# andimarafioti/qwen3-tts-cuda-graphs

Hardware: NVIDIA B200
Metric: audio_seconds_per_second (higher is better)
Workload: dtype bf16

## Files before the change

### include/fq3.h

```cpp
#ifndef FQ3_H_
#define FQ3_H_

#include <stdint.h>

#ifdef __cplusplus
extern "C" {
#endif

#define FQ3_ABI_VERSION 2
#define FQ3_MAX_CODE_GROUPS 32

typedef struct fq3_engine fq3_engine;

typedef struct fq3_stack_desc {
  int32_t hidden, inter, n_layers, n_q_heads, n_kv_heads, head_dim, vocab;
  float rms_eps;
  const uint64_t* layer_offs;
  uint64_t final_norm_off;
  uint64_t rope_cos_off, rope_sin_off;
  int32_t rope_len;
  int32_t max_pos;
} fq3_stack_desc;

typedef struct fq3_model_desc {
// ... 66 lines not shown
int fq3_prefill_head(fq3_engine* e, int stream_idx, const void* last_hidden, int T, const fq3_policy* policy, void* out_logits,
                     void* stream);
void* fq3_kv_cache_ptr(fq3_engine* e, int stream_idx, int layer, int which);
int fq3_talker_step(fq3_engine* e, int stream_idx, const void* embeds, int position, void* out_hidden,
                    void* out_logits, void* stream);
int fq3_predictor_run(fq3_engine* e, int stream_idx, const void* pred_input, const fq3_subpolicy* sub,
                      uint64_t seed, void* out_codes_i64, void* out_logits, void* stream);
int fq3_sample(fq3_engine* e, const void* logits_f32, int V, const void* history_i64, int n_history,
               const fq3_policy* policy, int eos_id, int suppress_eos, int flags, uint64_t draw_index,
               void* out_token_i64, void* stream);
int fq3_apply_repetition_penalty(fq3_engine* e, void* logits_f32, int V, const void* history_i64, int n_history,
                                 float penalty, int flags, void* stream);
int fq3_decode_frames(fq3_engine* e, int n_streams, int n_frames, const fq3_policy* policy,
                      const fq3_subpolicy* sub, void* stream);
int fq3_assemble_prompt(fq3_engine* e, const void* tp_rows, const void* desc_i32x4, int n_rows, const void* spk_rows,
                        const void* ref_codes_i32, void* out_bf16, void* stream);
int fq3_lockstep_group(const fq3_engine* e);

int fq3_reduced_grid(const fq3_engine* e);
int fq3_set_decode_grid(fq3_engine* e, int n_ctas);
int fq3_clear_fault(fq3_engine* e, void* stream);
int fq3_debug_set_epoch(fq3_engine* e, uint32_t epoch);
int fq3_debug_read_talker_logits(fq3_engine* e, int stream_idx, void* out_f32, void* stream);
int fq3_get_status(fq3_engine* e, int stream_idx, fq3_status* out, void* stream);
int fq3_read_codes(fq3_engine* e, int stream_idx, int first_frame, int n, int32_t* codes_out, void* stream);
int fq3_last_hidden(fq3_engine* e, int row, void* out_bf16, void* stream);
void* fq3_codes_device_ptr(fq3_engine* e, int stream_idx);

int fq3_debug_read_prof(fq3_engine* e, long long* out, int n_words);

int fq3_linear(fq3_engine* e, const void* W, const void* x, void* y, int M, int N, int K, int flags,
               const void* gamma, float eps, const void* bias, const void* residual, void* stream);

enum {
  FQ3_OK = 0,
  FQ3_E_INVALID = 1,
  FQ3_E_CUDA = 2,
  FQ3_E_TOO_LONG = 3,
  FQ3_E_DEVICE_FAULT = 4,
  FQ3_E_UNSUPPORTED = 5
};

#ifdef __cplusplus
}
#endif
#endif
// ... 1 lines not shown
```

### qwen3_tts_cuda_graphs_b200/_lib.py

```python
from __future__ import annotations

import ctypes as C
import os
import shutil

from . import build as _build


class StackDesc(C.Structure):
    _fields_ = [
        ("hidden", C.c_int32), ("inter", C.c_int32), ("n_layers", C.c_int32), ("n_q_heads", C.c_int32),
        ("n_kv_heads", C.c_int32), ("head_dim", C.c_int32), ("vocab", C.c_int32), ("rms_eps", C.c_float),
        ("layer_offs", C.POINTER(C.c_uint64)), ("final_norm_off", C.c_uint64),
        ("rope_cos_off", C.c_uint64), ("rope_sin_off", C.c_uint64), ("rope_len", C.c_int32), ("max_pos", C.c_int32),
    ]


class ModelDesc(C.Structure):
    _fields_ = [
        ("abi_version", C.c_int32), ("arena", C.c_void_p), ("arena_bytes", C.c_uint64),
        ("talker", StackDesc), ("predictor", StackDesc),
        ("codec_head_off", C.c_uint64), ("codec_embed_off", C.c_uint64), ("n_code_groups", C.c_int32),
        ("lm_head_offs", C.POINTER(C.c_uint64)), ("pred_embed_offs", C.POINTER(C.c_uint64)),
        ("has_s2m", C.c_int32), ("s2m_w_off", C.c_uint64), ("s2m_b_off", C.c_uint64),
# ... 35 lines not shown
    "fq3_set_stream_policy": (C.c_int, [_P, C.c_int, C.POINTER(Policy), _P]),
    "fq3_set_generation_state": (C.c_int, [_P, C.c_int, C.c_int, C.c_int, _P]),
    "fq3_set_text_conditioning": (C.c_int, [_P, C.c_int, _P, C.c_int, _P, _P]),
    "fq3_open_text": (C.c_int, [_P, C.c_int, _P, _P]),
    "fq3_append_text": (C.c_int, [_P, C.c_int, _P, C.c_int, C.c_int, _P]),
    "fq3_import_kv": (C.c_int, [_P, C.c_int, C.c_int, _P, _P, C.c_int, _P]),
    "fq3_set_loop_state": (C.c_int, [_P, C.c_int, C.c_int, _P, C.c_int, C.c_int, _P]),
    "fq3_prefill": (C.c_int, [_P, C.c_int, _P, C.c_int, C.c_int, C.POINTER(Policy), _P, _P]),
    "fq3_prefill_tail": (C.c_int, [_P, C.c_int, _P, C.c_int, C.c_int, C.POINTER(Policy), _P, _P]),
    "fq3_prefill_head": (C.c_int, [_P, C.c_int, _P, C.c_int, C.POINTER(Policy), _P, _P]),
    "fq3_kv_cache_ptr": (_P, [_P, C.c_int, C.c_int, C.c_int]),
    "fq3_talker_step": (C.c_int, [_P, C.c_int, _P, C.c_int, _P, _P, _P]),
    "fq3_predictor_run": (C.c_int, [_P, C.c_int, _P, C.POINTER(SubPolicy), C.c_uint64, _P, _P, _P]),
    "fq3_sample": (C.c_int, [_P, _P, C.c_int, _P, C.c_int, C.POINTER(Policy), C.c_int, C.c_int, C.c_int, C.c_uint64, _P, _P]),
    "fq3_apply_repetition_penalty": (C.c_int, [_P, _P, C.c_int, _P, C.c_int, C.c_float, C.c_int, _P]),
    "fq3_decode_frames": (C.c_int, [_P, C.c_int, C.c_int, C.POINTER(Policy), C.POINTER(SubPolicy), _P]),
    "fq3_reduced_grid": (C.c_int, [_P]),
    "fq3_lockstep_group": (C.c_int, [_P]),
    "fq3_assemble_prompt": (C.c_int, [_P, _P, _P, C.c_int, _P, _P, _P, _P]),
    "fq3_set_decode_grid": (C.c_int, [_P, C.c_int]),
    "fq3_clear_fault": (C.c_int, [_P, _P]),
    "fq3_debug_set_epoch": (C.c_int, [_P, C.c_uint32]),
    "fq3_debug_read_talker_logits": (C.c_int, [_P, C.c_int, _P, _P]),
    "fq3_get_status": (C.c_int, [_P, C.c_int, C.POINTER(Status), _P]),
    "fq3_read_codes": (C.c_int, [_P, C.c_int, C.c_int, C.c_int, C.POINTER(C.c_int32), _P]),
    "fq3_last_hidden": (C.c_int, [_P, C.c_int, _P, _P]),
    "fq3_codes_device_ptr": (_P, [_P, C.c_int]),
    "fq3_debug_read_prof": (C.c_int, [_P, C.POINTER(C.c_longlong), C.c_int]),
    "fq3_linear": (C.c_int, [_P, _P, _P, _P, C.c_int, C.c_int, C.c_int, C.c_int, _P, C.c_float, _P, _P, _P]),
}

_lib = None


class Fq3Error(RuntimeError):
    pass


def load():
    global _lib
    if _lib is not None:
        return _lib
    path = _build.lib_path("libfq3.so")
    if (not os.path.exists(path) or _build.is_stale("libfq3.so")) and (shutil.which("nvcc") or os.path.exists("/usr/local/cuda/bin/nvcc")):
        _build.build_lib("libfq3.so")
    if not os.path.exists(path):
# ... 24 lines not shown
```

### qwen3_tts_cuda_graphs_b200/csrc/fq3_api.cu

```cuda
#include <cstdio>
#include <cstdlib>
#include <cstring>
#include <string>
#include <array>
#include <vector>

#include "../../include/fq3.h"
#include "fq3_kernel.cuh"

using namespace fq3;

namespace {

thread_local std::string g_err;
int fail(int code, const std::string& msg) {
  g_err = msg;
  return -code;
}
#define CK(call)                                                                                     \
  do {                                                                                               \
    cudaError_t _e = (call);                                                                         \
    if (_e != cudaSuccess)                                                                           \
      return fail(FQ3_E_CUDA, std::string(#call) + ": " + cudaGetErrorString(_e) + " @" + __FILE__ + ":" + \
                                  std::to_string(__LINE__));                                         \
// ... 39 lines not shown
  uint8_t* seen_scratch = nullptr;
  Phase *d_frames = nullptr, *d_pred = nullptr, *d_talker = nullptr, *d_prefill = nullptr, *d_linear = nullptr, *d_wide = nullptr;
  std::vector<Phase> h_frames, h_pred, h_talker, h_prefill, h_wide;
  int n_frames_ph = 0, n_pred_ph = 0, n_talker_ph = 0, n_prefill_ph = 0, n_wide_ph = 0;
  int ref_stages = 0;
  int wide_rows = 0;
  std::vector<uint8_t> in_wpin;
  uint8_t* tiled = nullptr;
  size_t tiled_bytes = 0;
  std::vector<std::pair<uint64_t, uint64_t>> tiled_map;
  uint8_t* lin_img = nullptr;
  size_t lin_img_bytes = 0;
  size_t tiled_used = 0;
  int64_t launches = 0;
  long long* prof = nullptr;
  std::vector<Plan> plans;
  int n_sms = 0;
  std::vector<std::array<int, 3>> plan_keys;
  long ring_cap = 0;
  int prof_cta = -1;
  uint32_t epoch = 1;
  int lin_words = 0;
  unsigned long long watchdog_ns = 4000000000ull;
  std::vector<void*> owned;
};

namespace {

template <class T>
int dalloc(fq3_engine* e, T** p, size_t n, bool zero = true) {
  void* q = nullptr;
  CK(cudaMalloc(&q, std::max<size_t>(n * sizeof(T), 16)));
  if (zero) CK(cudaMemset(q, 0, std::max<size_t>(n * sizeof(T), 16)));
  e->owned.push_back(q);
  *p = reinterpret_cast<T*>(q);
  return 0;
}

uint32_t off16(uint64_t byte_off) { return (uint32_t)(byte_off >> 4); }

bool make_plan(int G, int N, int K, bool swiglu, Plan* out) {
  if (N < 2 || (N & 1) || K < 64 || (K % 64)) return false;
  if (swiglu && (N & 3)) return false;
  Plan pl{};
  pl.ro_shift = swiglu ? 2 : 1;
  const int n_groups = (N + kGroupRows - 1) / kGroupRows;
// ... 37 lines not shown
  p.w_off = off16(o[1]); p.g_off = off16(o[0]); p.b_off = 0; p.N = s.qkvdim(); p.K = s.d.hidden;
  p.plan = plan_id(e, p.N, p.K, false);
  v.push_back(p);
  p.type = PH_ATTN; p.flags = r2; p.in_buf = Q; p.out_buf = A; p.w_off = 0; p.g_off = off16(o[2]); p.b_off = off16(o[3]);
  p.N = 0; p.K = 0; p.plan = 0;
  v.push_back(p);
  p.type = PH_GEMV; p.flags = F_RESID | r2 | kp; p.in_buf = A; p.out_buf = X; p.res_buf = X;
  p.w_off = off16(o[4]); p.g_off = 0; p.b_off = 0; p.N = s.d.hidden; p.K = s.qdim();
  p.plan = plan_id(e, p.N, p.K, false);
  v.push_back(p);
  p.flags = F_PRENORM | F_SWIGLU | r2 | kp; p.in_buf = X; p.out_buf = C; p.res_buf = 0;
  p.w_off = off16(o[6]); p.g_off = off16(o[5]); p.N = 2 * s.d.inter; p.K = s.d.hidden;
  p.plan = plan_id(e, p.N, p.K, true);
  v.push_back(p);
  p.flags = F_RESID | r2 | kp; p.in_buf = C; p.out_buf = X; p.res_buf = X;
  p.w_off = off16(o[7]); p.g_off = 0; p.N = s.d.hidden; p.K = s.d.inter;
  p.plan = plan_id(e, p.N, p.K, false);
  v.push_back(p);
}

void push_predictor(std::vector<Phase>& v, fq3_engine* e, bool only) {
  for (int i = 0; i < e->ncb; ++i) {
    const bool r2 = (i == 0);
    if (e->desc.has_s2m) {
      Phase p{};
      p.type = PH_GEMV; p.stack = ST_PRED; p.aux = (uint8_t)i; p.flags = F_BIAS | F_L2_KEEP | (r2 ? F_ROWS2 : 0);
      p.in_buf = BUF_PIN; p.out_buf = BUF_PX; p.w_off = off16(e->desc.s2m_w_off); p.b_off = off16(e->desc.s2m_b_off);
      p.N = e->pr.d.hidden; p.K = e->tk.d.hidden;
      p.plan = plan_id(e, p.N, p.K, false);
      v.push_back(p);
    }
    for (int l = 0; l < e->pr.d.n_layers; ++l) push_layer(e, v, e->pr, ST_PRED, l, r2, (uint8_t)i, true);
    Phase h{};
    h.type = PH_GEMV; h.stack = ST_PRED; h.aux = (uint8_t)i;
    h.flags = F_PRENORM | F_OUT_F32 | F_L2_KEEP | (r2 ? F_ROWS2 : 0);
    h.in_buf = BUF_PX; h.out_buf = BUF_LOGITS; h.w_off = off16(e->lm_head_offs[i]);
    h.g_off = off16(e->pr.d.final_norm_off); h.N = e->pr.d.vocab; h.K = e->pr.d.hidden;
    h.plan = plan_id(e, h.N, h.K, false);
    v.push_back(h);
    Phase s{};
    s.type = PH_SAMPLE; s.stack = ST_PRED; s.aux = (uint8_t)i; s.skind = only ? SMP_PRED_ONLY : SMP_PRED;
    s.flags = r2 ? F_ROWS2 : 0;
    v.push_back(s);
  }
}

void push_predictor_wide(std::vector<Phase>& v, fq3_engine* e) {
  const int L = e->pr.d.n_layers;
  for (int half = 0; half < 2; ++half) {
    const uint16_t fb = half ? F_WPIN_B : 0;
    const size_t first = v.size();
    if (e->desc.has_s2m) {
      Phase p{};
      p.type = PH_GEMV; p.stack = ST_PRED; p.aux = 0; p.flags = F_BIAS | F_L2_KEEP | F_IN_PREV | fb;
      p.in_buf = BUF_WPIN; p.out_buf = BUF_PX; p.w_off = off16(e->desc.s2m_w_off); p.b_off = off16(e->desc.s2m_b_off);
// ... 84 lines not shown
  }
  if (dalloc(e, d, v.size(), false)) return -1;
  if (cudaMemcpy(*d, v.data(), v.size() * sizeof(Phase), cudaMemcpyHostToDevice) != cudaSuccess) return -1;
  return 0;
}

void fill_common(fq3_engine* e, LaunchParams& p) {
  p.arena = reinterpret_cast<const uint8_t*>(e->desc.arena);
  p.tiled = e->tiled;
  for (int i = 0; i < kNumBufs; ++i) { p.bufs[i] = e->bufs[i]; p.ld[i] = e->ld[i]; }
  p.stacks[0] = e->rt[0];
  p.stacks[1] = e->rt[1];
  p.st = e->d_st;
  p.attn_part = e->attn_part;
  for (size_t i = 0; i < e->plans.size(); ++i) p.plans[i] = e->plans[i];
  p.err = e->err_dev;
  p.n_code_groups = e->desc.n_code_groups;
  p.eos_id = e->desc.eos_id;
  p.has_s2m = e->desc.has_s2m;
  p.max_frames = e->desc.max_frames;
  p.codec_embed = reinterpret_cast<const bf16*>(p.arena + e->desc.codec_embed_off);
  for (int i = 0; i < e->ncb; ++i) p.pred_embeds[i] = reinterpret_cast<const bf16*>(p.arena + e->pred_embed_offs[i]);
  p.pred_logits_all = nullptr;
  p.pos_override = -1;
  p.watchdog_ns = e->watchdog_ns;
  p.debug = (16 << 16) | 32;
  p.prof = e->prof;
  p.prof_cta = e->prof_cta;
  if (const char* d = getenv("FQ3_DEBUG")) p.debug = atoi(d);
  p.n_iters = 1;
  p.stream0 = 0;
  p.wide = 0;
  p.max_streams = e->desc.max_streams;
}

int check_device_fault(fq3_engine* e) {
  if (e->err_host && e->err_host[0] != 0) {
    char b[256];
    snprintf(b, sizeof b, "device watchdog fault: code=%d cta=%d phase=%d detail=%d (1=grid barrier 2=ring full-wait "
                          "3=ring empty-wait 4=frame handshake 5=bad phase)",
             e->err_host[0], e->err_host[1], e->err_host[2], e->err_host[3]);
    return fail(FQ3_E_DEVICE_FAULT, b);
  }
  return 0;
}

// ... 115 lines not shown
  Policy p{};
  p.do_sample = q->do_sample; p.top_k = q->top_k; p.top_p = q->top_p; p.temperature = q->temperature;
  p.rep_pen = q->repetition_penalty; p.min_new_tokens = q->min_new_tokens; p.suppress_tail = q->suppress_tail;
  p.seed = q->seed;
  return p;
}
SubPolicy to_sub(const fq3_subpolicy* q) {
  SubPolicy p{};
  p.do_sample = q->do_sample; p.top_k = q->top_k; p.top_p = q->top_p; p.temperature = q->temperature;
  return p;
}

int sync_pin_layout(fq3_engine* e, int s0, int n, bool to_wpin, cudaStream_t s) {
  const int pb = e->desc.has_s2m ? BUF_PIN : BUF_PX;
  for (int i = s0; i < s0 + n; ++i) {
    if ((e->in_wpin[i] != 0) == to_wpin) continue;
    fq3_wpin_from_pairs_kernel<<<1, 256, 0, s>>>(reinterpret_cast<LLWord*>(e->bufs[BUF_WPIN]), e->ld[BUF_WPIN], reinterpret_cast<LLWord*>(e->bufs[pb]),
                                                 e->ld[pb], i, e->desc.max_streams, to_wpin ? 0 : 1);
    e->launches += 1;
    CK(cudaGetLastError());
    e->in_wpin[i] = to_wpin ? 1 : 0;
  }
  return 0;
}

int check_stack(const fq3_stack_desc& d, const char* name) {
  if (d.head_dim != kHeadDim) return fail(FQ3_E_UNSUPPORTED, std::string(name) + ": head_dim must be 128");
  if (d.hidden % 64 || d.inter % 64) return fail(FQ3_E_UNSUPPORTED, std::string(name) + ": dims must be multiples of 64");
  if (d.n_q_heads % d.n_kv_heads) return fail(FQ3_E_UNSUPPORTED, std::string(name) + ": nq % nkv != 0");
  if (d.n_q_heads / d.n_kv_heads > kGq) return fail(FQ3_E_UNSUPPORTED, std::string(name) + ": more than 2 q heads per kv head");
  if (d.vocab > kMaxVocab) return fail(FQ3_E_UNSUPPORTED, std::string(name) + ": vocab exceeds sampling scratch");
  if (d.vocab % 4) return fail(FQ3_E_UNSUPPORTED, std::string(name) + ": vocab must be a multiple of 4");
  return 0;
}

}

extern "C" {

int fq3_abi_version(void) { return FQ3_ABI_VERSION; }
const char* fq3_last_error(void) { return g_err.c_str(); }

static int create_impl(const fq3_model_desc* desc, fq3_engine* e);

int fq3_create(const fq3_model_desc* desc, fq3_engine** out) {
  if (!desc || !out) return fail(FQ3_E_INVALID, "null argument");
// ... 110 lines not shown
  e->text_open.assign(B, 0);
  if (dalloc(e, &e->d_st, B)) return -FQ3_E_CUDA;
  if (dalloc(e, &e->d_spol, B)) return -FQ3_E_CUDA;
  for (int b = 0; b < B; ++b) {
    StreamState& s = e->h_st[b];
    memset(&s, 0, sizeof s);
    bf16 *tr = nullptr, *pe = nullptr;
    if (dalloc(e, &tr, (size_t)e->tk.d.max_pos * Ht)) return -FQ3_E_CUDA;
    if (dalloc(e, &pe, (size_t)Ht)) return -FQ3_E_CUDA;
    if (dalloc(e, &s.held, (size_t)Ht)) return -FQ3_E_CUDA;
    if (dalloc(e, &s.codes, (size_t)desc->max_frames * desc->n_code_groups)) return -FQ3_E_CUDA;
    if (dalloc(e, &s.seen, (size_t)round_up(e->tk.d.vocab, 16))) return -FQ3_E_CUDA;
    s.trailing = tr;
    s.pad_embed = pe;
  }
  CK(cudaMemcpy(e->d_st, e->h_st.data(), sizeof(StreamState) * B, cudaMemcpyHostToDevice));
  auto gemv_bytes = [&](const StackHost& sh) {
    return (size_t)sh.d.n_layers * ((size_t)sh.qkvdim() * sh.d.hidden + (size_t)sh.d.hidden * sh.qdim() + 3ull * sh.d.hidden * sh.d.inter) * 2;
  };
  e->tiled_bytes = gemv_bytes(e->tk) + gemv_bytes(e->pr) + (size_t)e->tk.d.vocab * e->tk.d.hidden * 2 +
                   (size_t)e->ncb * e->pr.d.vocab * e->pr.d.hidden * 2 + (desc->has_s2m ? (size_t)e->pr.d.hidden * e->tk.d.hidden * 2 : 0) +
                   1024 * (size_t)(8 * (e->tk.d.n_layers + e->pr.d.n_layers) + e->ncb + 8);
  if (dalloc(e, &e->tiled, e->tiled_bytes, false)) return -FQ3_E_CUDA;
  std::vector<Phase>& v = e->h_frames;
  push_predictor(v, e, false);
  push_talker(v, e, false);
  {
    Phase s{};
    s.type = PH_SAMPLE; s.stack = ST_TALKER; s.skind = SMP_TALKER;
    v.push_back(s);
  }
  push_predictor(e->h_pred, e, true);
  push_talker(e->h_talker, e, false);
  push_talker(e->h_prefill, e, true);
  {
    Phase s{};
    s.type = PH_SAMPLE; s.stack = ST_TALKER; s.skind = SMP_PREFILL;
    e->h_prefill.push_back(s);
  }
  push_predictor_wide(e->h_wide, e);
  push_talker(e->h_wide, e, false);
  {
    Phase s{};
    s.type = PH_SAMPLE; s.stack = ST_TALKER; s.skind = SMP_TALKER;
    e->h_wide.push_back(s);
  }
// ... 1 lines not shown
  e->n_frames_ph = (int)e->h_frames.size();
  e->n_pred_ph = (int)e->h_pred.size();
  e->n_talker_ph = (int)e->h_talker.size();
  e->n_prefill_ph = (int)e->h_prefill.size();
  e->n_wide_ph = (int)e->h_wide.size();
  if (upload(e, e->h_wide, &e->d_wide)) return fail(FQ3_E_CUDA, "wide program upload");
  {
    const int kmax = std::max(e->tk.kmax(), e->pr.kmax());
    const long fixed = kHeaderBytes + kScratchBytes + (long)round_up((size_t)kKindBytes + kUnitBytes + (size_t)e->n_wide_ph * sizeof(Phase), 1024) +
                       (long)kGammaSlots * (long)round_up((size_t)std::max(e->tk.d.hidden, e->pr.d.hidden) * 2, 1024);
    const long spg_max = ((long)kmax * 16 + kStageBytes - 1) / kStageBytes;
    const long avail = (long)e->smem_max - fixed - std::max(4L, spg_max + 1) * kStageBytes - 2048;
    e->wide_rows = (int)std::max<long>(0, std::min<long>(avail / ((long)kmax * 2 + 64), kMaxWide));
  }
  {
    LaunchParams q{};
    q.n_phases = e->n_frames_ph; q.n_rows = 1;
    if (carve(e, q, e->h_frames.data()) < 0) return -FQ3_E_INVALID;
    e->ref_stages = q.n_stages;
  }
  if (upload(e, e->h_frames, &e->d_frames) || upload(e, e->h_pred, &e->d_pred) || upload(e, e->h_talker, &e->d_talker) ||
      upload(e, e->h_prefill, &e->d_prefill))
    return fail(FQ3_E_CUDA, "program upload / weight tiling (matrix rows must be a multiple of 8)");
  if (dalloc(e, &e->d_linear, 1)) return -FQ3_E_CUDA;
  CK(cudaDeviceSynchronize());
  return 0;
}

int fq3_destroy(fq3_engine* e) {
  if (!e) return 0;
  cudaDeviceSynchronize();
  for (void* p : e->owned) if (p) cudaFree(p);
  if (e->err_host) cudaFreeHost(e->err_host);
  delete e;
  return 0;
}

int fq3_num_sms(const fq3_engine* e) { return e ? e->G : 0; }
int64_t fq3_launch_count(const fq3_engine* e) { return e ? e->launches : 0; }

static int check_stream(fq3_engine* e, int idx) {
  if (!e) return fail(FQ3_E_INVALID, "null engine");
  if (idx < 0 || idx >= e->desc.max_streams) return fail(FQ3_E_INVALID, "stream index out of range");
  return 0;
}

// ... 325 lines not shown

int fq3_decode_frames(fq3_engine* e, int n_streams, int n_frames, const fq3_policy* policy, const fq3_subpolicy* sub,
                      void* stream) {
  if (!e || !policy || !sub) return fail(FQ3_E_INVALID, "bad decode arguments");
  if (n_streams < 1 || n_streams > e->desc.max_streams) return fail(FQ3_E_INVALID, "n_streams out of range");
  if (n_frames <= 0) return 0;
  int wide_from = 3;
  if (const char* wf = getenv("FQ3_WIDE_FROM")) wide_from = std::max(1, atoi(wf));
  if ((n_streams >= wide_from && e->wide_rows > kMaxRows / 2) || 2 * n_streams > kMaxRows) {
    if (e->wide_rows <= kMaxRows / 2)
      return fail(FQ3_E_UNSUPPORTED, "more than four lock-step streams do not fit this model's staging buffer: decode in groups of fq3_lockstep_group()");
    const int n_groups = (n_streams + e->wide_rows - 1) / e->wide_rows;
    const int per = (n_streams + n_groups - 1) / n_groups;
    if (int r = sync_pin_layout(e, 0, n_streams, true, (cudaStream_t)stream)) return r;
    for (int s0 = 0; s0 < n_streams; s0 += per) {
      const int n = std::min(per, n_streams - s0);
      if (int r = reserve_epochs(e, (uint64_t)n_frames * (uint64_t)e->n_wide_ph + 2, (cudaStream_t)stream)) return r;
      LaunchParams p{};
      fill_common(e, p);
      p.prog = e->d_wide;
      p.n_phases = e->n_wide_ph;
      p.mode = MODE_FRAMES;
      p.wide = 1;
      p.n_rows = n;
      p.stream0 = s0;
      p.n_iters = n_frames;
      p.pol = to_policy(policy);
      p.spol = spol_for(e, s0, n);
      p.sub = to_sub(sub);
      if (int r = launch(e, p, e->h_wide.data(), (cudaStream_t)stream)) return r;
    }
    return 0;
  }
  if (int r = reserve_epochs(e, (uint64_t)n_frames * (uint64_t)e->n_frames_ph + 2, (cudaStream_t)stream)) return r;
  if (int r = sync_pin_layout(e, 0, n_streams, false, (cudaStream_t)stream)) return r;
  LaunchParams p{};
  fill_common(e, p);
  p.prog = e->d_frames;
  p.n_phases = e->n_frames_ph;
  p.mode = MODE_FRAMES;
  p.n_rows = n_streams;
  p.n_iters = n_frames;
  p.pol = to_policy(policy);
  p.spol = spol_for(e, 0, n_streams);
  p.sub = to_sub(sub);
  return launch(e, p, e->h_frames.data(), (cudaStream_t)stream);
// ... 51 lines not shown
  return unpack_f32(e, out_f32, e->tk.d.vocab, BUF_LOGITS, idx, 1, e->tk.d.vocab, (cudaStream_t)stream);
}

int fq3_get_status(fq3_engine* e, int idx, fq3_status* out, void* stream) {
  if (int r = check_stream(e, idx)) return r;
  cudaError_t se = cudaStreamSynchronize((cudaStream_t)stream);
  if (int r = check_device_fault(e)) return r;
  if (se != cudaSuccess) return fail(FQ3_E_CUDA, std::string("stream sync: ") + cudaGetErrorString(se));
  StreamState s;
  CK(cudaMemcpy(&s, e->d_st + idx, sizeof s, cudaMemcpyDeviceToHost));
  out->n_frames = s.n_frames; out->done = s.done; out->position = s.position; out->gen_step = s.gen_step;
  out->token = s.token; out->error = e->err_host[0];
  return 0;
}

int fq3_read_codes(fq3_engine* e, int idx, int first, int n, int32_t* codes_out, void* stream) {
  if (int r = check_stream(e, idx)) return r;
  if (first < 0 || n < 0 || first + n > e->desc.max_frames) return fail(FQ3_E_INVALID, "frame range");
  if (n == 0) return 0;
  const int g = e->desc.n_code_groups;
  CK(cudaMemcpyAsync(codes_out, e->h_st[idx].codes + (size_t)first * g, (size_t)n * g * 4, cudaMemcpyDeviceToHost,
                     (cudaStream_t)stream));
  CK(cudaStreamSynchronize((cudaStream_t)stream));
  return 0;
}

int fq3_debug_read_prof(fq3_engine* e, long long* out, int n_words) {
  if (!e || !e->prof) return fail(FQ3_E_INVALID, "profiling not enabled (FQ3_PROF)");
  CK(cudaDeviceSynchronize());
  CK(cudaMemcpy(out, e->prof, sizeof(long long) * std::min(n_words, 512 * 160 * 2), cudaMemcpyDeviceToHost));
  CK(cudaMemset(e->prof, 0, sizeof(long long) * 512 * 160 * 2));
  return 0;
}

int fq3_last_hidden(fq3_engine* e, int row, void* out_bf16, void* stream) {
  if (!e || !out_bf16 || row < 0 || row >= e->max_rows) return fail(FQ3_E_INVALID, "bad arguments");
  const int Ht = e->tk.d.hidden;
  CK(cudaMemcpyAsync(out_bf16, reinterpret_cast<const bf16*>(e->bufs[BUF_HID]) + (size_t)row * e->ld[BUF_HID], (size_t)Ht * 2,
                     cudaMemcpyDeviceToDevice, (cudaStream_t)stream));
  return 0;
}

void* fq3_codes_device_ptr(fq3_engine* e, int idx) {
  if (!e || idx < 0 || idx >= e->desc.max_streams) return nullptr;
  return e->h_st[idx].codes;
}
// ... 56 lines not shown
```

### qwen3_tts_cuda_graphs_b200/csrc/fq3_common.cuh

```cuda
#pragma once
#include <cuda_bf16.h>
#include <cuda_runtime.h>
#include <stdint.h>

namespace fq3 {

typedef __nv_bfloat16 bf16;

constexpr int kConsumerWarps = 12;
constexpr int kConsumerThreads = kConsumerWarps * 32;
constexpr int kThreads = kConsumerThreads + 128;
constexpr int kProducerRegs = 56;
constexpr int kConsumerRegs = 152;
constexpr int kPollWarps = 8;
constexpr int kPollThreads = kPollWarps * 32;
constexpr int kMaxStages = 16;
constexpr int kGroupRows = 8;
constexpr int kChunkK = 32;
constexpr int kBlockBytes = kGroupRows * kChunkK * 2;
constexpr int kStageBytes = 16 * 1024;
constexpr int kStageChunks = kStageBytes / kBlockBytes;
constexpr int kHeadDim = 128;
constexpr int kMaxRows = 8;
constexpr int kMaxWide = 16;
// ... 15 lines not shown
constexpr int kGammaSlots = 4;
constexpr int kMaxPlans = 24;

typedef uint2 LLWord;

enum PhaseType : uint8_t { PH_END = 0, PH_GEMV = 1, PH_ATTN = 2, PH_SAMPLE = 3 };
enum StackId : uint8_t { ST_TALKER = 0, ST_PRED = 1 };
enum SampleKind : uint8_t { SMP_PRED = 0, SMP_TALKER = 1, SMP_PREFILL = 2, SMP_PRED_ONLY = 3 };

enum PhaseFlags : uint16_t {
  F_PRENORM = 1,
  F_BIAS = 2,
  F_RESID = 4,
  F_SWIGLU = 8,
  F_OUT_F32 = 16,
  F_ROWS2 = 32,
  F_LAST_ROW = 64,
  F_WRITE_NORMED = 128,
  F_L2_KEEP = 256,
  F_ABSPTR = 512,
  F_SILU = 1024,
  F_PASS0A = 2048,
  F_WPIN_B = 4096,
  F_IN_PREV = 8192
};

struct __align__(16) Phase {
  uint8_t type;
  uint8_t stack;
  uint8_t layer;
  uint8_t aux;
  uint16_t flags;
  uint8_t in_buf, out_buf;
  uint32_t w_off;
  uint32_t g_off;
  uint32_t b_off;
  uint32_t N;
  uint32_t K;
  uint8_t res_buf;
  uint8_t skind;
  uint8_t plan;
  uint8_t kind;
};
static_assert(sizeof(Phase) == 32, "Phase must stay 32 bytes");

enum BufId : uint8_t {
  BUF_TX = 0, BUF_TQKV, BUF_TATT, BUF_TACT, BUF_PX, BUF_PQKV, BUF_PATT, BUF_PACT, BUF_PIN,
// ... 89 lines not shown
  int n_iters;
  int mode;
  int n_rows;
  int wide;
  int max_streams;
  int stream0;
  int pos_override;
  int pf_pos0, pf_n_pad, pf_rope_delta, pf_final;
  const uint8_t* arena;
  const uint8_t* tiled;
  void* bufs[kNumBufs];
  int ld[kNumBufs];
  StackRt stacks[2];
  StreamState* st;
  Policy pol;
  SubPolicy sub;
  const StreamPolicy* spol;
  LLWord* attn_part;
  int* err;
  int n_code_groups, eos_id, has_s2m, max_frames;
  const bf16* codec_embed;
  const bf16* pred_embeds[32];
  float* pred_logits_all;
  const void* lin_W;
  const void* lin_gamma;
  const void* lin_bias;
  float lin_eps;
  int n_stages, xbuf_bytes, prog_bytes, gam_bytes;
  Plan plans[kMaxPlans];
  unsigned epoch_base;
  unsigned long long watchdog_ns;
  long long* prof;
  int prof_cta;
  int debug;
};

enum DevErr : int { DE_NONE = 0, DE_LL_WAIT = 1, DE_FULL_WAIT = 2, DE_EMPTY_WAIT = 3, DE_HANDSHAKE = 4, DE_BAD_PHASE = 5, DE_CTL_WAIT = 6, DE_ASSERT = 7 };

}
```

### qwen3_tts_cuda_graphs_b200/csrc/fq3_kernel.cuh

```cuda
#pragma once
#include "fq3_common.cuh"

namespace fq3 {

__device__ __forceinline__ uint32_t smem_u32(const void* p) { return (uint32_t)__cvta_generic_to_shared(p); }

__device__ __forceinline__ void mbar_init(uint64_t* bar, uint32_t count) {
  asm volatile("mbarrier.init.shared::cta.b64 [%0], %1;" ::"r"(smem_u32(bar)), "r"(count) : "memory");
}
__device__ __forceinline__ void mbar_arrive(uint64_t* bar) {
  asm volatile("mbarrier.arrive.shared::cta.b64 _, [%0];" ::"r"(smem_u32(bar)) : "memory");
}
__device__ __forceinline__ void mbar_arrive_expect_tx(uint64_t* bar, uint32_t bytes) {
  asm volatile("mbarrier.arrive.expect_tx.shared::cta.b64 _, [%0], %1;" ::"r"(smem_u32(bar)), "r"(bytes) : "memory");
}
__device__ __forceinline__ bool mbar_try_wait(uint64_t* bar, uint32_t parity) {
  uint32_t ok;
  asm volatile(
      "{\n\t.reg .pred p;\n\t"
      "mbarrier.try_wait.parity.shared::cta.b64 p, [%1], %2;\n\t"
      "selp.u32 %0, 1, 0, p;\n\t}"
      : "=r"(ok)
      : "r"(smem_u32(bar)), "r"(parity)
      : "memory");
// ... 509 lines not shown
  }
  cbar_sync();
  if (tprof) prof_acc(p, 2, *tprof);
}

template <int UNITS, int JC>
__device__ __noinline__ void load_x_rows(const LaunchParams& p, uint32_t flags, const LLWord* in, int ld, uint32_t gam, float eps,
                                         int K, int M, uint32_t ep_in, int pidx, uint32_t xs, uint32_t red) {
  load_x_rows_impl<UNITS, JC, false>(p, flags, in, ld, gam, eps, K, M, ep_in, pidx, xs, red, nullptr);
}

__device__ __forceinline__ float2 tree_parts(float y0, float y1, uint32_t pa, uint32_t stride, int wpg) {
  float P0[8], P1[8];
#pragma unroll
  for (int g = 0; g < 8; ++g) {
    float s0 = 0.f, s1 = 0.f;
    if (g != 0 && g < wpg) { const float2 v = lds_f32x2(pa + (uint32_t)g * stride); s0 = v.x; s1 = v.y; }
    if (g + 8 < wpg) { const float2 v = lds_f32x2(pa + (uint32_t)(g + 8) * stride); s0 += v.x; s1 += v.y; }
    if (g == 0) { s0 += y0; s1 += y1; }
    P0[g] = s0; P1[g] = s1;
  }
  return make_float2(((P0[0] + P0[1]) + (P0[2] + P0[3])) + ((P0[4] + P0[5]) + (P0[6] + P0[7])),
                     ((P1[0] + P1[1]) + (P1[2] + P1[3])) + ((P1[4] + P1[5]) + (P1[6] + P1[7])));
}

template <bool PROF>
__device__ __forceinline__ void gemv_phase_consume(const Ctx& c, const Phase& ph, const LaunchParams& p, RingCur& cur, RingCur& gcur, uint32_t& gst,
                                                   int pidx, uint32_t ep) {
  const int tid = threadIdx.x, warp = tid >> 5, lane = tid & 31;
  RingCur cur0 = cur, gcur0 = gcur;
  const uint32_t kda = c.kinds + (uint32_t)ph.kind * (uint32_t)sizeof(KindDesc);
  const uint4 k0 = lds128(kda);
  const uint4 k3 = lds128(kda + 48u);
  const uint4 ud = lds128(c.units + (uint32_t)(ph.kind * kConsumerWarps + warp) * (uint32_t)sizeof(UnitDesc));
  if (k3.x == 0u) return;
  const uint32_t flags = k0.w;
  const int Kq = (int)k0.z;
  const LLWord* in = reinterpret_cast<const LLWord*>(((unsigned long long)k0.y << 32) | k0.x);
  const uint32_t ep_in = (pidx == 0 && ep == p.epoch_base + 1) ? 0u : ep - 1;
  const bool norm = (flags & F_PRENORM) != 0;
  if (PROF) prof_mark(p, pidx, 0);
  if (PROF) prof_cta_time(p, pidx, 0);
  if (PROF) prof_warp_time(p, pidx, 0);

  const uint4 k6 = lds128(kda + 96u);
  const bool fast = k6.w != 0u;
// ... 24 lines not shown
  const uint32_t glap = gcur0.lap;
  if (norm) gcur0.advance(1, kGammaSlots);
  float eps = __uint_as_float(k5.x);
  float inv_k = __uint_as_float(k5.y);
  const uint32_t par = gst & 1u;
  const uint32_t xs = c.xs + (fast ? par * c.xhalf : 0u);
  uint32_t xdst0 = xs + xquad_off(tid), xdst1 = xs + xquad_off(tid + kPollThreads), xdst2 = xs + xquad_off(tid + 2 * kPollThreads);
  uint32_t xrow = xs + (uint32_t)min(g8, M - 1) * xrow_stride(K) + (uint32_t)t * 16u;
  const uint32_t lane_w = (uint32_t)lane * 16u;
  const uint32_t pbase = c.scratch + par * (uint32_t)(kConsumerWarps * 32 * 8);
  uint32_t pdst = pbase + (uint32_t)((wgrp * wpg + kp) * 32 + lane) * 8u;
  LLWord* out = reinterpret_cast<LLWord*>(((unsigned long long)k1.y << 32) | k1.x);
  const LLWord* resp = reinterpret_cast<const LLWord*>(((unsigned long long)k1.w << 32) | k1.z);
  const uint32_t* biasp = reinterpret_cast<const uint32_t*>(((unsigned long long)k2.y << 32) | k2.x);
  const int ldout = (int)k2.z, ldres = (int)k2.w;
  const bool f_lane = w_act && kp == 0 && g8 < M && (ro_shift == 1 || (t & 1) == 0);
  const int f_sub = (ro_shift == 1) ? t : (t >> 1);
  const int wpgrp = (int)k5.w;
  int gi = wgrp;
  int f_word = (sb.grp0 + gi) * wpgrp + f_sub;
  uint32_t res0 = 0u, bias0 = 0u;
  const bool g_ok0 = w_act && gi < sb.g;
  if (f_lane && g_ok0 && f_word < n_words) {
    if (flags & F_RESID) res0 = ll_ld(resp + (size_t)g8 * ldres + f_word).x;
    if (flags & F_BIAS) bias0 = __ldg(biasp + f_word);
  }
  RingCur my = cur0;
  const bool pre_ok = g_ok0;
  if (g_ok0) my.advance(gi * spg + (ch0 >> 5), c.n_stages);
  if (pre_ok) {
    if (!mbar_try_wait_a(c.full + (uint32_t)my.slot * 8u, my.lap)) {
      Spin spin;
      while (!mbar_try_wait_a(c.full + (uint32_t)my.slot * 8u, my.lap)) spin.tick(p, DE_FULL_WAIT, pidx, my.slot);
    }
  }
  int n_rounds = (int)k5.z;
  uint32_t wa0 = c.ring + lane_w + (uint32_t)my.slot * kStageBytes + (uint32_t)(ch0 & (kStageChunks - 1)) * kBlockBytes;
  uint32_t xa0 = xrow + (uint32_t)ch0 * kXBlock;
#ifndef FQ3_PRE
#define FQ3_PRE 0
#endif
  constexpr int kPre = FQ3_PRE > 0 ? FQ3_PRE : 1;
  uint4 wreg[kPre];
  int npre = 0;
  if (pre_ok && FQ3_PRE > 0) {
    npre = min(min(ch1, (ch0 | (kStageChunks - 1)) + 1) - ch0, kPre);
#pragma unroll
// ... 196 lines not shown
          for (int m = 0; m < M; ++m) {
            float s0 = 0.f, s1 = 0.f;
            const uint32_t q0 = pbase + (uint32_t)(wgrp * wpg * 32 + m * 4 + t) * 8u;
            if (g8 != 0 && g8 < wpg) { const float2 v = lds_f32x2(q0 + (uint32_t)g8 * 256u); s0 = v.x; s1 = v.y; }
            if (g8 + 8 < wpg) { const float2 v = lds_f32x2(q0 + (uint32_t)(g8 + 8) * 256u); s0 += v.x; s1 += v.y; }
            const float o0 = __shfl_sync(0xffffffffu, y0, m * 4 + t), o1 = __shfl_sync(0xffffffffu, y1, m * 4 + t);
            if (g8 == 0) { s0 += o0; s1 += o1; }
#pragma unroll
            for (int o = 4; o <= 16; o <<= 1) {
              s0 += __shfl_xor_sync(0xffffffffu, s0, o);
              s1 += __shfl_xor_sync(0xffffffffu, s1, o);
            }
            if (g8 == m) { r0 = s0; r1 = s1; }
          }
          y0 = r0; y1 = r1;
        }
      }
    }
    if (PROF && r == 0) prof_mark(p, pidx, 10, kProfLeader);
    if (kp == 0) {
      if (r != 0) {
        f_word = (sb.grp0 + gi) * wpgrp + f_sub;
        if (f_lane && f_word < n_words) {
          if (flags & F_RESID) res0 = ll_ld(resp + (size_t)g8 * ldres + f_word).x;
          if (flags & F_BIAS) bias0 = __ldg(biasp + f_word);
        }
      }
      float lo, hi;
      if (flags & F_SWIGLU) {
        const float e = bf16r(bf16r(silu_f(bf16r(y0))) * bf16r(y1));
        lo = e;
        hi = __shfl_down_sync(0xffffffffu, e, 1);
      } else {
        lo = y0; hi = y1;
        if (flags & F_BIAS) { lo += bf_lo(bias0); hi += bf_hi(bias0); }
        lo = bf16r(lo); hi = bf16r(hi);
        if (flags & F_SILU) { lo = bf16r(silu_f(lo)); hi = bf16r(silu_f(hi)); }
      }
      if (flags & F_RESID) { lo = bf16r(bf_lo(res0) + lo); hi = bf16r(bf_hi(res0) + hi); }
      if (PROF) prof_cta_time(p, pidx, 1);
      if (f_lane && f_word < n_words) ll_st(out + (size_t)g8 * ldout + f_word, pack_bf16x2(lo, hi), ep);
      if (PROF && r == 0) prof_mark(p, pidx, 11, kProfLeader);
      if (PROF && r == 0) prof_warp_time(p, pidx, 7);
      if (wpg == 1) {
        __syncwarp();
        if (lane == 0) {
          int rs = cur0.slot + gi * spg;
// ... 1474 lines not shown
    int pick = -1;
#pragma unroll
    for (int j = 0; j < 8; ++j) {
      if (e[j] > 0.f && (pick < 0 || target >= c)) { pick = 8 * tid + j; }
      c += e[j];
    }
    if (pick >= 0) atomicMin(&redi[20], pick);
  }
  cbar_sync();
  int tok = redi[20];
  if (tok == 0x7fffffff) tok = imax;
  prof_mark(*lp, pidx, 5);
  return tok;
}

__device__ __forceinline__ int sample_ll(const LLWord* ll, uint32_t ep, const LaunchParams& p, int pidx, const SampleArgs& a, unsigned char* scratch) {
  if (a.top_p >= 1.0f && a.V <= 8 * kConsumerThreads && (a.V & 3) == 0) return sample_fast(ll, ep, &p, pidx, a, scratch);
  return sample_row(nullptr, ll, ep, &p, pidx, a, sample_scratch(scratch));
}

__device__ __forceinline__ void publish_row(LLWord* dst, const bf16* src, int n, uint32_t ep) {
  for (int c = threadIdx.x; c < (n >> 1); c += kConsumerThreads) ll_st(dst + c, __ldg(reinterpret_cast<const uint32_t*>(src) + c), ep);
}
__device__ __noinline__ void publish_held_row(LLWord* dst, const bf16* src, int n, uint32_t ep) {
  for (int c = threadIdx.x; c < (n >> 1); c += kConsumerThreads) ll_st(dst + c, __ldcg(reinterpret_cast<const uint32_t*>(src) + c), ep);
}
__device__ __noinline__ void hold_row(bf16* dst, const bf16* src, int n) {
  for (int c = threadIdx.x; c < (n >> 1); c += kConsumerThreads)
    __stcg(reinterpret_cast<uint32_t*>(dst) + c, __ldg(reinterpret_cast<const uint32_t*>(src) + c));
}

template <bool WIDE>
__device__ __forceinline__ void sample_phase(const Phase& ph, const LaunchParams& p, unsigned char* smem_base, uint32_t ep, int pidx,
                             const int* frame_done) {
  const Smem sm = carve_smem(smem_base, p);
  const SampleScratch sc = sample_scratch(sm.scratch);
  const int Ht = p.stacks[ST_TALKER].hidden;
  const int ncb = p.n_code_groups - 1;
  const uint32_t ep_in = ep - 1;
  if ((int)blockIdx.x >= (p.mode == MODE_PREFILL ? 1 : p.n_rows) && threadIdx.x == 0 && ph.skind != SMP_PRED && ph.skind != SMP_PRED_ONLY)
    __threadfence();
  for (int b = blockIdx.x; b < (p.mode == MODE_PREFILL ? 1 : p.n_rows); b += gridDim.x) {
    prof_mark(p, pidx, 0);
    cbar_sync();
    const int slot = p.stream0 + b;
    StreamState* st = p.st + slot;
// ... 1 lines not shown
    LLWord* pin = reinterpret_cast<LLWord*>(p.bufs[p.has_s2m ? BUF_PIN : BUF_PX]);
    const int ldpin = p.ld[p.has_s2m ? BUF_PIN : BUF_PX];
    const LLWord* lgbuf = reinterpret_cast<const LLWord*>(p.bufs[BUF_LOGITS]);
    if (ph.skind == SMP_PRED || ph.skind == SMP_PRED_ONLY) {
      const int i = ph.aux;
      const int Vp = p.stacks[ST_PRED].vocab;
      const int lrow = (ph.flags & F_ROWS2) ? 2 * b + 1 : b;
      const LLWord* lg = lgbuf + (size_t)lrow * p.ld[BUF_LOGITS];
      if (p.pred_logits_all) {
        for (int v = threadIdx.x; v < (Vp >> 1); v += kConsumerThreads) {
          const uint32_t pay = ll_wait(lg + v, ep_in, p, pidx);
          p.pred_logits_all[(size_t)i * Vp + 2 * v] = bf_lo(pay);
          p.pred_logits_all[(size_t)i * Vp + 2 * v + 1] = bf_hi(pay);
        }
      }
      const bool own = p.spol != nullptr && __ldcg(&p.spol[slot].on) != 0;
      const unsigned long long seed = own ? __ldcg(&p.spol[slot].pol.seed) : p.pol.seed;
      SampleArgs a;
      a.V = Vp; a.do_sample = p.sub.do_sample; a.top_k = p.sub.top_k; a.top_p = p.sub.top_p;
      a.temperature = p.sub.temperature; a.rep_pen = 1.0f; a.seen = nullptr; a.suppress_start = Vp; a.eos = -1;
      a.suppress_eos = 0; a.round_bf16 = 1; a.seed = seed ^ (0x9E3779B97F4A7C15ull * (unsigned long long)(own ? 1 : slot + 1));
      a.draw = __ldcg(&st->draws) + (unsigned long long)(i + 1);
      a.next_emb = p.pred_embeds[i]; a.emb_row_bytes = Ht * 2;
      const int tok = sample_ll(lg, ep_in, p, pidx, a, sm.scratch);
      FQ3_ASSERT(tok >= 0 && tok < Vp, pidx, 100000 + tok);
      if (threadIdx.x == 0) st->cur_codes[i + 1] = tok;
      if (i + 1 < ncb) {
        publish_row(pin + (size_t)b * ldpin, p.pred_embeds[i] + (size_t)tok * Ht, Ht, ep);
      } else if (ph.skind == SMP_PRED) {
        const int nfr = __ldcg(&st->n_frames);
        const int c0 = __ldcg(&st->token);
        if (!done) {
          if (threadIdx.x < p.n_code_groups && nfr < p.max_frames) {
            const int code = (threadIdx.x == 0) ? c0 : (threadIdx.x == ncb ? tok : __ldcg(&st->cur_codes[threadIdx.x]));
            st->codes[(size_t)nfr * p.n_code_groups + threadIdx.x] = code;
          }
          if (threadIdx.x == 0) {
            st->n_frames = nfr + 1;
            st->seen[c0] = 1;
            st->draws = __ldcg(&st->draws) + 32ull;
          }
        }
        cbar_sync();
        const int gs = __ldcg(&st->gen_step);
        const int ntr = __ldcg(&st->n_trailing);
        const bf16* text = (gs < ntr) ? st->trailing + (size_t)gs * Ht : st->pad_embed;
        LLWord* tx = reinterpret_cast<LLWord*>(p.bufs[BUF_TX]) + (size_t)b * p.ld[BUF_TX];
        const uint32_t* ce = reinterpret_cast<const uint32_t*>(p.codec_embed + (size_t)c0 * Ht);
        const uint32_t* tx32 = reinterpret_cast<const uint32_t*>(text);
        for (int c = threadIdx.x; c < (Ht >> 1); c += kConsumerThreads) {
// ... 409 lines not shown
```

Before: 46.12.

## Precompute predictor layer-0 QKV per codebook token and skip that GEMV

At engine creation, builds a table holding the predictor's layer-0 QKV projection for every codebook embedding row. During decode the sampler publishes the table row for the chosen token straight into the QKV buffer, and the layer-0 QKV GEMV phase is removed for codebooks after the first. The following phase now waits on an epoch two steps back for its residual. This trades extra device memory and a one-time build for one fewer weight-streaming GEMV and phase barrier per codebook step. It also tightens the epoch and ordering assumptions between the sampler and the next phase.

```diff
diff --git a/include/fq3.h b/include/fq3.h
--- a/include/fq3.h
+++ b/include/fq3.h
@@ -112,6 +112,7 @@
 int fq3_clear_fault(fq3_engine* e, void* stream);
 int fq3_debug_set_epoch(fq3_engine* e, uint32_t epoch);
 int fq3_debug_read_talker_logits(fq3_engine* e, int stream_idx, void* out_f32, void* stream);
+int fq3_debug_read_pred_qkv_table(fq3_engine* e, int codebook, int token, void* out_bf16, void* stream);
 int fq3_get_status(fq3_engine* e, int stream_idx, fq3_status* out, void* stream);
 int fq3_read_codes(fq3_engine* e, int stream_idx, int first_frame, int n, int32_t* codes_out, void* stream);
 int fq3_last_hidden(fq3_engine* e, int row, void* out_bf16, void* stream);
diff --git a/qwen3_tts_cuda_graphs_b200/_lib.py b/qwen3_tts_cuda_graphs_b200/_lib.py
--- a/qwen3_tts_cuda_graphs_b200/_lib.py
+++ b/qwen3_tts_cuda_graphs_b200/_lib.py
@@ -81,6 +81,7 @@
     "fq3_clear_fault": (C.c_int, [_P, _P]),
     "fq3_debug_set_epoch": (C.c_int, [_P, C.c_uint32]),
     "fq3_debug_read_talker_logits": (C.c_int, [_P, C.c_int, _P, _P]),
+    "fq3_debug_read_pred_qkv_table": (C.c_int, [_P, C.c_int, C.c_int, _P, _P]),
     "fq3_get_status": (C.c_int, [_P, C.c_int, C.POINTER(Status), _P]),
     "fq3_read_codes": (C.c_int, [_P, C.c_int, C.c_int, C.c_int, C.POINTER(C.c_int32), _P]),
     "fq3_last_hidden": (C.c_int, [_P, C.c_int, _P, _P]),
diff --git a/qwen3_tts_cuda_graphs_b200/csrc/fq3_api.cu b/qwen3_tts_cuda_graphs_b200/csrc/fq3_api.cu
--- a/qwen3_tts_cuda_graphs_b200/csrc/fq3_api.cu
+++ b/qwen3_tts_cuda_graphs_b200/csrc/fq3_api.cu
@@ -85,6 +85,8 @@
   uint32_t epoch = 1;
   int lin_words = 0;
   unsigned long long watchdog_ns = 4000000000ull;
+  bool qkv_table = false;
+  bf16* pred_qkv_table = nullptr;
   std::vector<void*> owned;
 };
 
@@ -168,6 +170,7 @@
 void push_predictor(std::vector<Phase>& v, fq3_engine* e, bool only) {
   for (int i = 0; i < e->ncb; ++i) {
     const bool r2 = (i == 0);
+    const size_t at = v.size();
     if (e->desc.has_s2m) {
       Phase p{};
       p.type = PH_GEMV; p.stack = ST_PRED; p.aux = (uint8_t)i; p.flags = F_BIAS | F_L2_KEEP | (r2 ? F_ROWS2 : 0);
@@ -177,6 +180,10 @@
       v.push_back(p);
     }
     for (int l = 0; l < e->pr.d.n_layers; ++l) push_layer(e, v, e->pr, ST_PRED, l, r2, (uint8_t)i, true);
+    if (e->qkv_table && i > 0) {
+      v.erase(v.begin() + at);
+      v[at + 1].flags |= F_RES_WAIT;
+    }
     Phase h{};
     h.type = PH_GEMV; h.stack = ST_PRED; h.aux = (uint8_t)i;
     h.flags = F_PRENORM | F_OUT_F32 | F_L2_KEEP | (r2 ? F_ROWS2 : 0);
@@ -307,6 +314,7 @@
   p.codec_embed = reinterpret_cast<const bf16*>(p.arena + e->desc.codec_embed_off);
   for (int i = 0; i < e->ncb; ++i) p.pred_embeds[i] = reinterpret_cast<const bf16*>(p.arena + e->pred_embed_offs[i]);
   p.pred_logits_all = nullptr;
+  p.pred_qkv_table = e->pred_qkv_table;
   p.pos_override = -1;
   p.watchdog_ns = e->watchdog_ns;
   p.debug = (16 << 16) | 32;
@@ -468,6 +476,42 @@
     e->in_wpin[i] = to_wpin ? 1 : 0;
   }
   return 0;
+}
+
+int build_pred_qkv_table(fq3_engine* e) {
+  const int Ht = e->tk.d.hidden, Vp = e->pr.d.vocab, qkv = e->pr.qkvdim(), ntab = e->ncb - 1;
+  size_t q0 = 0;
+  while (q0 < e->h_frames.size() && !(e->h_frames[q0].type == PH_GEMV && e->h_frames[q0].stack == ST_PRED)) ++q0;
+  if (q0 == e->h_frames.size() || e->h_frames[q0].out_buf != BUF_PQKV || e->h_frames[q0].in_buf != BUF_PX)
+    return fail(FQ3_E_INVALID, "layer-0 qkv phase of the predictor not found");
+  Phase ph = e->h_frames[q0];
+  ph.flags &= (uint16_t)~F_ROWS2;
+  ph.kind = 0;
+  Phase* d_prog = nullptr;
+  if (dalloc(e, &d_prog, 1, false)) return -FQ3_E_CUDA;
+  CK(cudaMemcpy(d_prog, &ph, sizeof ph, cudaMemcpyHostToDevice));
+  if (dalloc(e, &e->pred_qkv_table, (size_t)ntab * Vp * qkv, false)) return -FQ3_E_CUDA;
+  const uint8_t* arena = reinterpret_cast<const uint8_t*>(e->desc.arena);
+  cudaStream_t s = 0;
+  for (int i = 0; i < ntab; ++i) {
+    const bf16* emb = reinterpret_cast<const bf16*>(arena + e->pred_embed_offs[i]);
+    for (int t0 = 0; t0 < Vp; t0 += kMaxRows) {
+      const int m = std::min(kMaxRows, Vp - t0);
+      if (int r = reserve_epochs(e, 3, s)) return r;
+      if (int r = pack_ll(e, BUF_PX, 0, emb + (size_t)t0 * Ht, Ht, m, Ht, s)) return r;
+      LaunchParams p{};
+      fill_common(e, p);
+      p.pred_qkv_table = nullptr;
+      p.prog = d_prog;
+      p.n_phases = 1;
+      p.mode = MODE_PREDICTOR;
+      p.n_rows = m;
+      if (int r = launch(e, p, &ph, s)) return r;
+      if (int r = unpack_bf16(e, e->pred_qkv_table + ((size_t)i * Vp + t0) * qkv, qkv, BUF_PQKV, 0, m, qkv, s)) return r;
+    }
+  }
+  CK(cudaDeviceSynchronize());
+  return check_device_fault(e);
 }
 
 int check_stack(const fq3_stack_desc& d, const char* name) {
@@ -624,6 +668,8 @@
                    (size_t)e->ncb * e->pr.d.vocab * e->pr.d.hidden * 2 + (desc->has_s2m ? (size_t)e->pr.d.hidden * e->tk.d.hidden * 2 : 0) +
                    1024 * (size_t)(8 * (e->tk.d.n_layers + e->pr.d.n_layers) + e->ncb + 8);
   if (dalloc(e, &e->tiled, e->tiled_bytes, false)) return -FQ3_E_CUDA;
+  const char* tq = getenv("FQ3_PRED_QKV_TABLE");
+  e->qkv_table = !desc->has_s2m && e->ncb > 1 && !(tq && atoi(tq) == 0);
   std::vector<Phase>& v = e->h_frames;
   push_predictor(v, e, false);
   push_talker(v, e, false);
@@ -671,6 +717,8 @@
   if (upload(e, e->h_frames, &e->d_frames) || upload(e, e->h_pred, &e->d_pred) || upload(e, e->h_talker, &e->d_talker) ||
       upload(e, e->h_prefill, &e->d_prefill))
     return fail(FQ3_E_CUDA, "program upload / weight tiling (matrix rows must be a multiple of 8)");
+  if (e->qkv_table)
+    if (int r = build_pred_qkv_table(e)) return r;
   if (dalloc(e, &e->d_linear, 1)) return -FQ3_E_CUDA;
   CK(cudaDeviceSynchronize());
   return 0;
@@ -1042,6 +1090,7 @@
       p.n_phases = e->n_wide_ph;
       p.mode = MODE_FRAMES;
       p.wide = 1;
+      p.pred_qkv_table = nullptr;
       p.n_rows = n;
       p.stream0 = s0;
       p.n_iters = n_frames;
@@ -1139,6 +1188,16 @@
   CK(cudaMemcpyAsync(codes_out, e->h_st[idx].codes + (size_t)first * g, (size_t)n * g * 4, cudaMemcpyDeviceToHost,
                      (cudaStream_t)stream));
   CK(cudaStreamSynchronize((cudaStream_t)stream));
+  return 0;
+}
+
+int fq3_debug_read_pred_qkv_table(fq3_engine* e, int codebook, int token, void* out_bf16, void* stream) {
+  if (!e || !out_bf16) return fail(FQ3_E_INVALID, "bad arguments");
+  if (!e->pred_qkv_table) return fail(FQ3_E_UNSUPPORTED, "this engine has no predictor q/k/v table (small_to_mtp model or FQ3_PRED_QKV_TABLE=0)");
+  if (codebook < 0 || codebook >= e->ncb - 1 || token < 0 || token >= e->pr.d.vocab) return fail(FQ3_E_INVALID, "row out of range");
+  const size_t qkv = (size_t)e->pr.qkvdim();
+  CK(cudaMemcpyAsync(out_bf16, e->pred_qkv_table + ((size_t)codebook * e->pr.d.vocab + token) * qkv, qkv * 2, cudaMemcpyDeviceToDevice,
+                     (cudaStream_t)stream));
   return 0;
 }
 
diff --git a/qwen3_tts_cuda_graphs_b200/csrc/fq3_common.cuh b/qwen3_tts_cuda_graphs_b200/csrc/fq3_common.cuh
--- a/qwen3_tts_cuda_graphs_b200/csrc/fq3_common.cuh
+++ b/qwen3_tts_cuda_graphs_b200/csrc/fq3_common.cuh
@@ -61,7 +61,8 @@
   F_SILU = 1024,
   F_PASS0A = 2048,
   F_WPIN_B = 4096,
-  F_IN_PREV = 8192
+  F_IN_PREV = 8192,
+  F_RES_WAIT = 16384
 };
 
 struct __align__(16) Phase {
@@ -197,6 +198,7 @@
   const bf16* codec_embed;
   const bf16* pred_embeds[32];
   float* pred_logits_all;
+  const bf16* pred_qkv_table;
   const void* lin_W;
   const void* lin_gamma;
   const void* lin_bias;
diff --git a/qwen3_tts_cuda_graphs_b200/csrc/fq3_kernel.cuh b/qwen3_tts_cuda_graphs_b200/csrc/fq3_kernel.cuh
--- a/qwen3_tts_cuda_graphs_b200/csrc/fq3_kernel.cuh
+++ b/qwen3_tts_cuda_graphs_b200/csrc/fq3_kernel.cuh
@@ -555,6 +555,11 @@
   }
   return make_float2(((P0[0] + P0[1]) + (P0[2] + P0[3])) + ((P0[4] + P0[5]) + (P0[6] + P0[7])),
                      ((P1[0] + P1[1]) + (P1[2] + P1[3])) + ((P1[4] + P1[5]) + (P1[6] + P1[7])));
+}
+
+__device__ __forceinline__ uint32_t res_word(const LLWord* ptr, uint32_t flags, uint32_t ep, const LaunchParams& p, int pidx) {
+  const LLWord w = ll_ld(ptr);
+  return (flags & F_RES_WAIT) ? ll_check(w, ptr, ep - 2u, p, pidx) : w.x;
 }
 
 template <bool PROF>
@@ -625,7 +630,7 @@
   uint32_t res0 = 0u, bias0 = 0u;
   const bool g_ok0 = w_act && gi < sb.g;
   if (f_lane && g_ok0 && f_word < n_words) {
-    if (flags & F_RESID) res0 = ll_ld(resp + (size_t)g8 * ldres + f_word).x;
+    if (flags & F_RESID) res0 = res_word(resp + (size_t)g8 * ldres + f_word, flags, ep, p, pidx);
     if (flags & F_BIAS) bias0 = __ldg(biasp + f_word);
   }
   RingCur my = cur0;
@@ -868,7 +873,7 @@
       if (r != 0) {
         f_word = (sb.grp0 + gi) * wpgrp + f_sub;
         if (f_lane && f_word < n_words) {
-          if (flags & F_RESID) res0 = ll_ld(resp + (size_t)g8 * ldres + f_word).x;
+          if (flags & F_RESID) res0 = res_word(resp + (size_t)g8 * ldres + f_word, flags, ep, p, pidx);
           if (flags & F_BIAS) bias0 = __ldg(biasp + f_word);
         }
       }
@@ -2389,6 +2394,21 @@
 __device__ __forceinline__ void publish_row(LLWord* dst, const bf16* src, int n, uint32_t ep) {
   for (int c = threadIdx.x; c < (n >> 1); c += kConsumerThreads) ll_st(dst + c, __ldg(reinterpret_cast<const uint32_t*>(src) + c), ep);
 }
+__device__ __noinline__ void publish_row16(LLWord* dst, const bf16* src, int n, uint32_t ep) {
+  const uint4* s4 = reinterpret_cast<const uint4*>(src);
+  const int q = n >> 3;
+  for (int c = threadIdx.x; c < q; c += 2 * kConsumerThreads) {
+    const int c1 = c + kConsumerThreads;
+    const uint4 v0 = __ldg(s4 + c);
+    const uint4 v1 = (c1 < q) ? __ldg(s4 + c1) : make_uint4(0u, 0u, 0u, 0u);
+    ll_st2(dst + 4 * c, v0.x, v0.y, ep);
+    ll_st2(dst + 4 * c + 2, v0.z, v0.w, ep);
+    if (c1 < q) {
+      ll_st2(dst + 4 * c1, v1.x, v1.y, ep);
+      ll_st2(dst + 4 * c1 + 2, v1.z, v1.w, ep);
+    }
+  }
+}
 __device__ __noinline__ void publish_held_row(LLWord* dst, const bf16* src, int n, uint32_t ep) {
   for (int c = threadIdx.x; c < (n >> 1); c += kConsumerThreads) ll_st(dst + c, __ldcg(reinterpret_cast<const uint32_t*>(src) + c), ep);
 }
@@ -2436,10 +2456,13 @@
       a.suppress_eos = 0; a.round_bf16 = 1; a.seed = seed ^ (0x9E3779B97F4A7C15ull * (unsigned long long)(own ? 1 : slot + 1));
       a.draw = __ldcg(&st->draws) + (unsigned long long)(i + 1);
       a.next_emb = p.pred_embeds[i]; a.emb_row_bytes = Ht * 2;
+      const bf16* tab = (p.pred_qkv_table && i + 1 < ncb) ? p.pred_qkv_table + (size_t)i * Vp * (2 * p.ld[BUF_PQKV]) : nullptr;
       const int tok = sample_ll(lg, ep_in, p, pidx, a, sm.scratch);
       FQ3_ASSERT(tok >= 0 && tok < Vp, pidx, 100000 + tok);
       if (threadIdx.x == 0) st->cur_codes[i + 1] = tok;
       if (i + 1 < ncb) {
+        if (tab) publish_row16(reinterpret_cast<LLWord*>(p.bufs[BUF_PQKV]) + (size_t)b * p.ld[BUF_PQKV], tab + (size_t)tok * (2 * p.ld[BUF_PQKV]),
+                               2 * p.ld[BUF_PQKV], ep);
         publish_row(pin + (size_t)b * ldpin, p.pred_embeds[i] + (size_t)tok * Ht, Ht, ep);
       } else if (ph.skind == SMP_PRED) {
         const int nfr = __ldcg(&st->n_frames);
```

Result: faster. 46.61 (median of 6 runs) (+1.1%).
